# tfwcn/tensorflow2-machine-vision

Hardware: NVIDIA B200
Metric: images/sec (higher is better)
Workload: dtype f32

## Files before the change

### tensorflow2-machine-vision_b200/csrc/yolo_loss.cu

```cuda
#include "yolo_targets.cuh"
#include "exchange.cuh"

#define YL_LEVELS 3
#define YL_CHUNK 256
#define YL_ICHUNK 128

enum { YL_VARIANT_TF_YOLO_UTILS = 0, YL_VARIANT_KERAS_YOLO3 = 1 };

struct YlLevels {
  const float* y_true[YL_LEVELS];
  const float* y_pred[YL_LEVELS];
  int h[YL_LEVELS], w[YL_LEVELS], rec_per_img[YL_LEVELS], anchor_base[YL_LEVELS];
  int chunks_per_img[YL_LEVELS];
  int cta_base[YL_LEVELS + 1];
  int obj_chunks_per_img[YL_LEVELS];
  int obj_cta_base[YL_LEVELS + 1];
  uint32_t magic_w[YL_LEVELS];
  float anc_w[YL_LEVELS][8], anc_h[YL_LEVELS][8];
};

struct YlParams {
  YlLevels lv;
  int B, A, C, RF, n_img;
  float img_w, img_h;
  float thr;
  int metric, variant;
  float* obj_compact;
  float4* gt_box;
  float4* gt_aux;
  float log_thr;
  float logk[YL_LEVELS][8];
  float tmin_w[YL_LEVELS][8], tmin_h[YL_LEVELS][8];
  uint32_t magic_a;
  float* conf_grad;
  int32_t* obj_index;
  float inv_div;
  unsigned char* out_ignore;
  const float4* sp_t;
  const int32_t* sp_cls;
  const uint32_t* obj_bits;
  int bits_words;
  int32_t* gt_count;
  unsigned int* scan_ticket;
  uint32_t* pend_queue;
  unsigned int* pend_count;
  unsigned long long* obj_fixed;
  double* partials;
  double* partials_obj;
};

__device__ __forceinline__ void yl_locate(const YlLevels& lv, int cta, int& l, int& img, int& chunk) {
  l = 0;
#pragma unroll
  for (int k = 1; k < YL_LEVELS; ++k) if (cta >= lv.cta_base[k]) l = k;
  const int r = cta - lv.cta_base[l];
  img = r / lv.chunks_per_img[l];
  chunk = r - img * lv.chunks_per_img[l];
}

__device__ __forceinline__ bool yl_regular(const BoxT& b) {
  return (b.c2 > b.c0) && (b.c3 > b.c1) && (b.area > 0.0f) && (b.area < 3.0e38f) && (b.at == b.at) &&
         (dm_fabsf(b.c0) < 3.0e38f) && (dm_fabsf(b.c1) < 3.0e38f) && (dm_fabsf(b.c2) < 3.0e38f) && (dm_fabsf(b.c3) < 3.0e38f);
}

#define YL_OBJ_PER_THREAD 4
#define YL_OBJ_CHUNK (YL_CHUNK * YL_OBJ_PER_THREAD)

#define YL_SORT_CAP 2048
__device__ __forceinline__ void yl_gtprep_body(const YlParams& p, int l, int img, int* s_idx) {
  const int nthr = blockDim.x;
  const int rpi = p.lv.rec_per_img[l];
  const float* yt = p.sp_t ? nullptr : p.lv.y_true[l] + ((size_t)img * rpi) * p.RF;
  const int n = __ldcg(&p.gt_count[img * YL_LEVELS + l]);
  const size_t gbase = (size_t)img * p.n_img + p.lv.anchor_base[l];
  if (!p.sp_t && n > 1 && n <= YL_SORT_CAP) {
    for (int k = threadIdx.x; k < n; k += nthr) s_idx[k] = __ldcg(&p.obj_index[gbase + k]);
    __syncthreads();
    for (int k = threadIdx.x; k < n; k += nthr) {
      const int mine = s_idx[k];
      int rank = 0;
      for (int j = 0; j < n; ++j) rank += (s_idx[j] < mine) ? 1 : 0;
      p.obj_index[gbase + rank] = mine;
// ... 368 lines not shown
  if (n_gt > 0) {
    if (threadIdx.x == 0) s_nq = 0;
    if (threadIdx.x < YL_ICHUNK / 32) s_hit[threadIdx.x] = 0u;
    s_t[threadIdx.x] = make_float4(tx, ty, tw, th);
    __syncthreads();
    const YlFilter f = yl_filter_init(p, l, rin, active, tx, ty, tw, th);
    yl_filter_gts(f, gbox, gaux, n_gt, [&](int g, const float4 c, const float4 x, bool rejected) {
      if (!active | hit | rejected) return;
      const int slot = atomicAdd(&s_nq, 1);
      if (slot < YL_QCAP) s_q[slot] = (threadIdx.x << 24) | (uint32_t)g;
      else {
        float otx = tx, oty = ty, otw = tw, oth = th;
        asm volatile("" : "+f"(otx), "+f"(oty), "+f"(otw), "+f"(oth));
        if (yl_pair_hits(p, l, rin, otx, oty, otw, oth, c, x)) hit = true;
      }
    });
    if (hit) atomicOr(&s_hit[warp], 1u << lane);
    __syncthreads();
    const int nq = min(s_nq, YL_QCAP);
    for (int q = threadIdx.x; q < nq; q += YL_ICHUNK) {
      const uint32_t e = s_q[q];
      const int r = (int)(e >> 24), g = (int)(e & 0xffffffu);
      if ((s_hit[r >> 5] >> (r & 31)) & 1u) continue;
      const float4 t = s_t[r];
      if (yl_pair_hits(p, l, chunk * YL_ICHUNK + r, t.x, t.y, t.z, t.w, __ldg(gbox + g), __ldg(gaux + g)))
        atomicOr(&s_hit[r >> 5], 1u << (r & 31));
    }
    __syncthreads();
    hit = (s_hit[warp] >> lane) & 1u;
  }
  float e = 0.f;
  if (active) e = yl_record_term(p, l, img, p.lv.anchor_base[l] + rin, obj, pobj, hit, false);
  yl_store_partial(p, icta, e, s_acc);
}

#define YL_FIXED_ONE 4294967296.0

__global__ void __launch_bounds__(YL_ICHUNK, 10) yolo_loss_ignore_lean_kernel(YlParams p) {
  __shared__ double s_acc[YL_ICHUNK / 32];
  const int n_term_cta = YL_LEVELS * p.B * YL_TERM_SPLIT;
  const int n_icta = (int)gridDim.x - n_term_cta;
  if ((int)blockIdx.x >= n_icta) {
    __shared__ double s_tacc[YL_ICHUNK / 32][3];
    yl_terms_body(p, blockIdx.x - n_icta, s_tacc);
    return;
  }
  const int icta = blockIdx.x;
  int l, img, chunk;
  yl_locate(p.lv, icta, l, img, chunk);
  const int rpi = p.lv.rec_per_img[l];
  const int rin = chunk * YL_ICHUNK + (int)threadIdx.x;
  const int lane = threadIdx.x & 31;
  const bool active = rin < rpi;
  const int n_gt = p.gt_count[img * YL_LEVELS + l];
  const float4* gbox = p.gt_box + (size_t)img * p.n_img + p.lv.anchor_base[l];
  const float4* gaux = p.gt_aux + (size_t)img * p.n_img + p.lv.anchor_base[l];
  float obj = 0.f, tx = 0.f, ty = 0.f, tw = 0.f, th = 0.f, pobj = 0.f;
  if (active) {
    obj = yl_obj(p, img, p.lv.anchor_base[l] + rin);
    const size_t f0 = ((size_t)img * rpi + rin) * p.RF;
    const float4 lo = __ldcg(reinterpret_cast<const float4*>(p.lv.y_pred[l]) + (f0 >> 2));
    const float4 hi = __ldcg(reinterpret_cast<const float4*>(p.lv.y_pred[l]) + (f0 >> 2) + 1);
    yl_rotate5(lo, hi, (int)(f0 & 3), tx, ty, tw, th, pobj);
  }
  bool pending = false;
  if (n_gt > 0) {
    const YlFilter f = yl_filter_init(p, l, rin, active, tx, ty, tw, th);
    yl_filter_gts(f, gbox, gaux, n_gt, [&](int, const float4, const float4, bool rejected) { pending |= active & !rejected; });
  }
  {
    const uint32_t pm = __ballot_sync(0xffffffffu, pending);
    if (pm) {
      unsigned int base = 0;
      if (lane == 0) base = atomicAdd(p.pend_count, (unsigned int)__popc(pm));
      base = __shfl_sync(0xffffffffu, base, 0);
      if (pending) p.pend_queue[base + __popc(pm & ((1u << lane) - 1u))] = (uint32_t)((size_t)img * p.n_img + p.lv.anchor_base[l] + rin);
    }
  }
  float e = 0.f;
  if (active && !pending) e = yl_record_term(p, l, img, p.lv.anchor_base[l] + rin, obj, pobj, false, true);
  yl_store_partial(p, icta, e, s_acc);
}

__device__ __forceinline__ void yl_exact_pass(const YlParams& p, unsigned int gwarp, unsigned int nwarps) {
  const int lane = threadIdx.x & 31;
  const int half = lane >> 4, sub = lane & 15;
  const unsigned int n = *p.pend_count;
  for (unsigned int q0 = gwarp * 2u; q0 < n; q0 += nwarps * 2u) {
    const unsigned int q = q0 + (unsigned int)half;
    const bool valid = q < n;
    const uint32_t id = valid ? p.pend_queue[q] : 0u;
    const int img = (int)(id / (uint32_t)p.n_img);
    const int ain = (int)(id - (uint32_t)img * (uint32_t)p.n_img);
    int l = 0;
#pragma unroll
    for (int k = 1; k < YL_LEVELS; ++k) if (ain >= p.lv.anchor_base[k]) l = k;
    const int rin = ain - p.lv.anchor_base[l];
    const int rpi = p.lv.rec_per_img[l];
    const float* rec = p.lv.y_pred[l] + ((size_t)img * rpi + rin) * p.RF;
    const float tx = __ldg(rec), ty = __ldg(rec + 1), tw = __ldg(rec + 2), th = __ldg(rec + 3), pobj = __ldg(rec + 4);
    const float obj = yl_obj(p, img, ain);
    const int n_gt = valid ? p.gt_count[img * YL_LEVELS + l] : 0;
    const float4* gbox = p.gt_box + (size_t)img * p.n_img + p.lv.anchor_base[l];
    const float4* gaux = p.gt_aux + (size_t)img * p.n_img + p.lv.anchor_base[l];
    const BoxT pb = yl_decode_record(p, l, rin, tx, ty, tw, th);
    const bool pb_regular = yl_regular(pb);
    bool hit = false;
    for (int g0 = 0;; g0 += 16) {
      const bool more = g0 < n_gt && !hit;
      if (!__any_sync(0xffffffffu, more)) break;
      const int g = g0 + sub;
      bool h = false;
      if (more && g < n_gt) h = yl_box_hits(p, pb, pb_regular, __ldg(gbox + g), __ldg(gaux + g));
      const uint32_t bal = __ballot_sync(0xffffffffu, h);
      hit = hit || ((bal >> (16 * half)) & 0xffffu) != 0u;
    }
    if (valid && sub == 0) {
      const float e = yl_record_term(p, l, img, ain, obj, pobj, hit, false);
      if (e == e && e < 1.0e9f) atomicAdd(p.obj_fixed + l, (unsigned long long)((double)e * YL_FIXED_ONE + 0.5));
      else atomicOr(p.obj_fixed + l, 0x8000000000000000ull);
    }
  }
}

__global__ void __launch_bounds__(128) yolo_loss_ignore_exact_kernel(YlParams p) {
  yl_exact_pass(p, blockIdx.x * (blockDim.x >> 5) + (threadIdx.x >> 5), gridDim.x * (blockDim.x >> 5));
}

#define YL_FIN_CTAS 32
#define YL_FIN_THREADS 256

struct YlFinalize {
  const double* partials; const double* partials_obj;
  int cta_base[YL_LEVELS + 1]; int obj_cta_base[YL_LEVELS + 1];
  float batch_divisor; float* parts; float* loss;
  double* slices;
  unsigned int* ticket;
  B200Exchange xchg;
  const unsigned long long* obj_fixed;
  int publish_only;
};

__global__ void __launch_bounds__(YL_FIN_THREADS) yolo_loss_finalize_kernel(YlFinalize f, YlParams p, int exact) {
  __shared__ double s_red[YL_FIN_THREADS / 32][12];
  __shared__ bool s_last;
  if (exact) yl_exact_pass(p, blockIdx.x * (YL_FIN_THREADS / 32) + (threadIdx.x >> 5), gridDim.x * (YL_FIN_THREADS / 32));
  if ((int)blockIdx.x >= YL_FIN_CTAS) {
    __syncthreads();
    if (threadIdx.x == 0) { __threadfence(); s_last = (atomicAdd(f.ticket, 1u) == gridDim.x - 1); }
    __syncthreads();
    if (!s_last) return;
  } else {
  double acc[12];
#pragma unroll
  for (int i = 0; i < 12; ++i) acc[i] = 0.0;
  const int t0 = blockIdx.x * YL_FIN_THREADS + (int)threadIdx.x, stride = YL_FIN_CTAS * YL_FIN_THREADS;
#pragma unroll
  for (int l = 0; l < 3; ++l) {
#pragma unroll 4
    for (int c = f.cta_base[l] + t0; c < f.cta_base[l + 1]; c += stride) acc[l * 4 + 2] += f.partials[c];
    for (int c = f.obj_cta_base[l] + t0; c < f.obj_cta_base[l + 1]; c += stride) {
      acc[l * 4 + 0] += f.partials_obj[(size_t)c * 3 + 0];
      acc[l * 4 + 1] += f.partials_obj[(size_t)c * 3 + 1];
      acc[l * 4 + 3] += f.partials_obj[(size_t)c * 3 + 2];
    }
  }
  const int lane_ = threadIdx.x & 31, warp_ = threadIdx.x >> 5;
#pragma unroll
  for (int i = 0; i < 12; ++i) {
    double v = warp_sum_d(acc[i]);
    if (lane_ == 0) s_red[warp_][i] = v;
  }
  __syncthreads();
  if (threadIdx.x < 12) {
    double s = 0.0;
    for (int w = 0; w < YL_FIN_THREADS / 32; ++w) s += s_red[w][threadIdx.x];
    f.slices[blockIdx.x * 12 + threadIdx.x] = s;
    __threadfence();
  }
  __syncthreads();
  if (threadIdx.x == 0) { __threadfence(); s_last = (atomicAdd(f.ticket, 1u) == gridDim.x - 1); }
  __syncthreads();
  if (!s_last) return;
  }
  __threadfence();
  const int lane = threadIdx.x & 31, warp = threadIdx.x >> 5;
  if (warp == 0) {
    float v = 0.0f;
    if (lane < 12) {
      double s = 0.0;
      for (int g = 0; g < YL_FIN_CTAS; ++g) s += __ldcg(f.slices + g * 12 + lane);
      if (f.obj_fixed && (lane & 3) == 2) {
        const unsigned long long fx = __ldcg(f.obj_fixed + (lane >> 2));
        s += (fx >> 63) ? (double)__longlong_as_double(0x7ff8000000000000ll) : (double)fx * (1.0 / YL_FIXED_ONE);
      }
      v = DM_DIV((float)s, f.batch_divisor);
    }
    if (f.publish_only && f.xchg.world > 1) xchg_publish_warp<float>(f.xchg, v, 12);
    else v = xchg_allreduce_warp<float>(f.xchg, v, 12);
    if (lane < 12 && f.parts) f.parts[lane] = v;
    float total = 0.0f;
    for (int l = 0; l < 3; ++l) {
      const float t0_ = __shfl_sync(0xffffffffu, v, l * 4 + 0), t1 = __shfl_sync(0xffffffffu, v, l * 4 + 1);
      const float t2 = __shfl_sync(0xffffffffu, v, l * 4 + 2), t3 = __shfl_sync(0xffffffffu, v, l * 4 + 3);
      total = DM_ADD(total, DM_ADD(DM_ADD(DM_ADD(t0_, t1), t2), t3));
    }
    if (lane == 0) { *f.loss = total; *f.ticket = 0u; }
  }
}

struct YlGradDense {
  float* grad[YL_LEVELS];
  const float* conf_grad[YL_LEVELS];
  unsigned long long quads[YL_LEVELS];
  unsigned long long records[YL_LEVELS];
  int RF;
};

__global__ void __launch_bounds__(256) yolo_loss_grad_dense_kernel(YlGradDense g) {
  const int lane = threadIdx.x & 31;
  const unsigned long long total = g.quads[YL_LEVELS - 1];
  const unsigned long long wstride = (unsigned long long)gridDim.x * (blockDim.x >> 5);
  const int RF = g.RF;
  for (unsigned long long w = (unsigned long long)blockIdx.x * (blockDim.x >> 5) + (threadIdx.x >> 5); w < total; w += wstride) {
    unsigned long long q = w;
    const float* cg = g.conf_grad[0];
    float* gr = g.grad[0];
    if (w >= g.quads[1]) { q = w - g.quads[1]; cg = g.conf_grad[2]; gr = g.grad[2]; }
    else if (w >= g.quads[0]) { q = w - g.quads[0]; cg = g.conf_grad[1]; gr = g.grad[1]; }
    const float mine = (lane < 4) ? __ldg(cg + q * 4ull + lane) : 0.0f;
    const float c0 = __shfl_sync(0xffffffffu, mine, 0), c1 = __shfl_sync(0xffffffffu, mine, 1);
    const float c2 = __shfl_sync(0xffffffffu, mine, 2), c3 = __shfl_sync(0xffffffffu, mine, 3);
    float4* dst = reinterpret_cast<float4*>(gr) + q * (unsigned long long)RF;
    for (int j = lane; j < RF; j += 32) {
      const int e = 4 * j;
      float v[4];
#pragma unroll
      for (int k = 0; k < 4; ++k) {
        const int x = e + k - 4;
        v[k] = (x == 0) ? c0 : (x == RF) ? c1 : (x == 2 * RF) ? c2 : (x == 3 * RF) ? c3 : 0.0f;
      }
      __stcs(dst + j, make_float4(v[0], v[1], v[2], v[3]));
    }
  }
  if (blockIdx.x == 0) {
#pragma unroll
    for (int l = 0; l < YL_LEVELS; ++l) {
      const unsigned long long r0 = g.records[l] & ~3ull, n_tail = (g.records[l] - r0) * (unsigned long long)RF;
      for (unsigned long long t = threadIdx.x; t < n_tail; t += blockDim.x) {
        const unsigned long long rec = r0 + t / (unsigned long long)RF;
        const int c = (int)(t % (unsigned long long)RF);
        g.grad[l][r0 * (unsigned long long)RF + t] = (c == 4) ? g.conf_grad[l][rec] : 0.0f;
      }
    }
  }
}

#define YL_GRAD_SPLIT 8
__global__ void __launch_bounds__(256) yolo_loss_grad_objects_kernel(YlParams p, float* g0, float* g1, float* g2) {
  const int pair = blockIdx.x / YL_GRAD_SPLIT, split = blockIdx.x - pair * YL_GRAD_SPLIT;
  const int img = pair / YL_LEVELS, l = pair - img * YL_LEVELS;
  float* grad = (l == 0 ? g0 : l == 1 ? g1 : g2);
  const int n = p.gt_count[img * YL_LEVELS + l];
  const int rpi = p.lv.rec_per_img[l];
  const int lane = threadIdx.x & 31, warp = threadIdx.x >> 5;
  const int W = p.lv.w[l], H = p.lv.h[l];
  const float* yt = p.lv.y_true[l] + ((size_t)img * rpi) * p.RF;
  const float* yp = p.lv.y_pred[l] + ((size_t)img * rpi) * p.RF;
// ... 189 lines not shown
  for (int l = 0; l < YL_LEVELS; ++l)
    for (int a = 0; a < A; ++a)
    {
      p.logk[l][a] = (float)log(((double)p.lv.anc_w[l][a] * (double)p.lv.anc_h[l][a]) / ((double)img_w * (double)img_h));
      const double tw = log(4e-5 * (double)img_w / (double)p.lv.anc_w[l][a]);
      const double th = log(4e-5 * (double)img_h / (double)p.lv.anc_h[l][a]);
      p.tmin_w[l][a] = (float)(tw > -6.0 ? tw : -6.0);
      p.tmin_h[l][a] = (float)(th > -6.0 ? th : -6.0);
    }
  p.out_ignore = out_ignore;
  p.inv_div = 1.0f / batch_divisor;
  p.conf_grad = out_grad ? reinterpret_cast<float*>(wsb + ws.cgrad) : nullptr;
  p.obj_index = reinterpret_cast<int32_t*>(wsb + ws.oidx);
  p.magic_a = A == 1 ? 0u : (uint32_t)((1ull << 32) / (unsigned long long)A + 1ull);
  for (int l = 0; l < YL_LEVELS; ++l) p.lv.magic_w[l] = p.lv.w[l] == 1 ? 0u : (uint32_t)((1ull << 32) / (unsigned long long)p.lv.w[l] + 1ull);
  p.gt_count = reinterpret_cast<int32_t*>(wsb + ws.cnt);
  p.partials = reinterpret_cast<double*>(wsb + ws.part);
  p.partials_obj = reinterpret_cast<double*>(wsb + ws.part_obj);
  if (stages & 1) B200_CUDA(cudaMemsetAsync(wsb + ws.cnt, 0, ws.cnt_bytes, stream));
  p.pend_queue = reinterpret_cast<uint32_t*>(wsb + ws.pend);
  p.pend_count = reinterpret_cast<unsigned int*>(wsb + ws.cnt) + (size_t)B * YL_LEVELS + 1;
  p.obj_fixed = reinterpret_cast<unsigned long long*>(wsb + ws.cnt + b200_align_up(sizeof(int32_t) * ((size_t)B * YL_LEVELS + 2), 8));
  p.scan_ticket = (!sparse && (stages & 3) == 3) ? reinterpret_cast<unsigned int*>(p.obj_fixed + 3) : nullptr;
  p.sp_t = nullptr; p.sp_cls = nullptr; p.obj_bits = nullptr; p.bits_words = 0;
  if (sparse) {
    B200_REQUIRE(sparse->total_boxes >= 0 && sparse->offsets && sparse->assign_anchors_wh_host, B200_ERR_BAD_ARG, "b200_yolo_loss_from_boxes: null box arrays");
    B200_REQUIRE(sparse->total_boxes == 0 || (sparse->boxes && sparse->classes), B200_ERR_BAD_ARG, "b200_yolo_loss_from_boxes: null box arrays");
    B200_REQUIRE((reinterpret_cast<uintptr_t>(sparse->boxes) & 15) == 0, B200_ERR_BAD_ARG, "b200_yolo_loss_from_boxes: boxes not 16-byte aligned");
    YtParams t;
    B200_REQUIRE(yt_fill_geometry(t, A, C, sparse->assign_anchors_wh_host, image_wh_host, hw) == 0, B200_ERR_BAD_ARG, "b200_yolo_loss_from_boxes: bad geometry");
    t.boxes = sparse->boxes; t.classes = sparse->classes; t.offsets = sparse->offsets; t.B = B; t.total = sparse->total_boxes;
    p.bits_words = sws.bits_words;
    float4* sp_t = reinterpret_cast<float4*>(wsb + sws.sp_t);
    int32_t* sp_cls = reinterpret_cast<int32_t*>(wsb + sws.sp_cls);
    uint32_t* bits = reinterpret_cast<uint32_t*>(wsb + sws.bits);
    if (stages & 1) {
      B200_CUDA(cudaMemsetAsync(bits, 0, sizeof(uint32_t) * (size_t)B * sws.bits_words, stream));
      yolo_loss_assign_sparse_kernel<<<B, 128, 0, stream>>>(t, p, reinterpret_cast<int*>(wsb + sws.keys), sp_t, sp_cls, bits);
      B200_LAUNCH_CHECK();
    }
    p.sp_t = sp_t; p.sp_cls = sp_cls; p.obj_bits = bits;
  } else if (stages & 1) {
    yolo_loss_scan_kernel<<<ws.n_cta_obj, YL_CHUNK, 0, stream>>>(p);
    B200_LAUNCH_CHECK();
  }
  if ((stages & 2) && !p.scan_ticket) {
    yolo_loss_gtprep_kernel<<<YL_LEVELS * B, 128, 0, stream>>>(p);
    B200_LAUNCH_CHECK();
  }
  bool use_split = false;
  if (stages & 4) {
    cudaPointerAttributes attr;
    bool host_pred = false;
    if (cudaPointerGetAttributes(&attr, y_pred[YL_LEVELS - 1]) == cudaSuccess) host_pred = attr.type == cudaMemoryTypeHost;
    else (void)cudaGetLastError();
    const int grid = YL_LEVELS * B * YL_TERM_SPLIT + ws.n_cta;
    bool aligned16 = true;
    for (int l = 0; l < YL_LEVELS; ++l) aligned16 &= (reinterpret_cast<uintptr_t>(y_pred[l]) & 15) == 0;
    use_split = !host_pred && aligned16 && p.RF >= 8;
    if (use_split) {
      if (!(stages & 1)) B200_CUDA(cudaMemsetAsync(p.pend_count, 0, (size_t)(reinterpret_cast<unsigned char*>(p.obj_fixed + 3) - reinterpret_cast<unsigned char*>(p.pend_count)), stream));
      yolo_loss_ignore_lean_kernel<<<grid, YL_ICHUNK, 0, stream>>>(p);
      if (!(stages & 8)) {
        B200_LAUNCH_CHECK();
        yolo_loss_ignore_exact_kernel<<<1024, 128, 0, stream>>>(p);
      }
    } else {
      yolo_loss_ignore_kernel<<<grid, YL_ICHUNK, 0, stream>>>(p);
    }
    B200_LAUNCH_CHECK();
  }
  if (!(stages & 8)) return B200_OK;
  YlFinalize f;
  f.partials = p.partials; f.partials_obj = p.partials_obj;
  for (int l = 0; l <= YL_LEVELS; ++l) { f.cta_base[l] = p.lv.cta_base[l]; f.obj_cta_base[l] = l * B * YL_TERM_SPLIT; }
  f.batch_divisor = batch_divisor; f.parts = out_parts; f.loss = out_loss;
  f.slices = reinterpret_cast<double*>(wsb + ws.fin);
  f.ticket = reinterpret_cast<unsigned int*>(wsb + ws.cnt) + (size_t)B * YL_LEVELS;
  f.publish_only = publish_only;
  f.obj_fixed = p.obj_fixed;
  if (xchg) f.xchg = *xchg;
  else { f.xchg.rank = 0; f.xchg.world = 1; for (int r = 0; r < B200_XCHG_MAX_WORLD; ++r) f.xchg.mailbox[r] = nullptr; }
  int wide = 4 * b200_sm_count();
  if (wide < YL_FIN_CTAS) wide = YL_FIN_CTAS;
  yolo_loss_finalize_kernel<<<use_split ? wide : YL_FIN_CTAS, YL_FIN_THREADS, 0, stream>>>(f, p, use_split ? 1 : 0);
  B200_LAUNCH_CHECK();
  if (out_grad) {
    YlGradDense g;
    g.RF = p.RF;
    unsigned long long cum = 0;
    for (int l = 0; l < YL_LEVELS; ++l) {
      B200_REQUIRE(out_grad[l] && (reinterpret_cast<uintptr_t>(out_grad[l]) & 15) == 0, B200_ERR_BAD_ARG, "b200_yolo_loss_grad: grad level %d null or not 16-byte aligned", l);
      g.records[l] = (unsigned long long)B * p.lv.rec_per_img[l];
      g.grad[l] = out_grad[l];
      g.conf_grad[l] = p.conf_grad + (size_t)B * p.lv.anchor_base[l];
      cum += g.records[l] / 4ull;
      g.quads[l] = cum;
    }
    unsigned long long blocks = (cum + 7) / 8;
    const unsigned long long cap = (unsigned long long)b200_sm_count() * 64;
    if (blocks > cap) blocks = cap;
    if (blocks < 1) blocks = 1;
    yolo_loss_grad_dense_kernel<<<(int)blocks, 256, 0, stream>>>(g);
    B200_LAUNCH_CHECK();
    yolo_loss_grad_objects_kernel<<<B * YL_LEVELS * YL_GRAD_SPLIT, 256, 0, stream>>>(p, out_grad[0], out_grad[1], out_grad[2]);
    B200_LAUNCH_CHECK();
  }
  return B200_OK;
}

extern "C" int b200_yolo_loss(const float* const y_true[3], const float* const y_pred[3], const int32_t hw[6], int B,
                              int A, int C, const float* anchors_wh_host, const float* image_wh_host,
                              float iou_thresh, int metric, int variant, float batch_divisor, float* out_parts,
                              float* out_loss, unsigned char* out_ignore, void* workspace, size_t workspace_bytes,
                              void* stream_) {
  return yolo_loss_impl(y_true, y_pred, hw, B, A, C, anchors_wh_host, image_wh_host, iou_thresh, metric, variant,
                        batch_divisor, out_parts, out_loss, out_ignore, nullptr, workspace, workspace_bytes, stream_);
}

extern "C" int b200_yolo_loss_stages(const float* const y_true[3], const float* const y_pred[3], const int32_t hw[6], int B,
                                     int A, int C, const float* anchors_wh_host, const float* image_wh_host,
                                     float iou_thresh, int metric, int variant, float batch_divisor, float* out_parts,
                                     float* out_loss, void* workspace, size_t workspace_bytes, int stages, void* stream_) {
  B200_REQUIRE(stages > 0 && stages <= 0xf, B200_ERR_BAD_ARG, "b200_yolo_loss_stages: stages must be a non-empty subset of 0xf");
  return yolo_loss_impl(y_true, y_pred, hw, B, A, C, anchors_wh_host, image_wh_host, iou_thresh, metric, variant,
                        batch_divisor, out_parts, out_loss, nullptr, nullptr, workspace, workspace_bytes, stream_, nullptr, stages);
}

extern "C" size_t b200_yolo_loss_from_boxes_workspace_bytes(const int32_t hw[6], int B, int A, int total_boxes) {
  int n_img = 0;
  const YlWs w = yl_layout(hw, B, A, &n_img, nullptr);
  return yl_sparse_layout(w.total, B, n_img, total_boxes).total;
}

extern "C" int b200_yolo_loss_from_boxes(const float* boxes, const int32_t* classes, const int32_t* offsets, int total_boxes,
                                         const float* assign_anchors_wh_host, const float* const y_pred[3], const int32_t hw[6],
                                         int B, int A, int C, const float* anchors_wh_host, const float* image_wh_host,
                                         float iou_thresh, int metric, int variant, float batch_divisor, float* out_parts,
                                         float* out_loss, unsigned char* out_ignore, void* workspace, size_t workspace_bytes,
                                         void* stream_) {
  YlSparseIn sp;
  sp.boxes = boxes; sp.classes = classes; sp.offsets = offsets; sp.total_boxes = total_boxes;
  sp.assign_anchors_wh_host = assign_anchors_wh_host;
  return yolo_loss_impl(nullptr, y_pred, hw, B, A, C, anchors_wh_host, image_wh_host, iou_thresh, metric, variant,
                        batch_divisor, out_parts, out_loss, out_ignore, nullptr, workspace, workspace_bytes, stream_, &sp);
}

extern "C" int b200_yolo_loss_grad(const float* const y_true[3], const float* const y_pred[3], const int32_t hw[6],
                                   int B, int A, int C, const float* anchors_wh_host, const float* image_wh_host,
                                   float iou_thresh, int metric, int variant, float batch_divisor, float* out_parts,
                                   float* out_loss, float* const out_grad[3], void* workspace, size_t workspace_bytes,
                                   void* stream_) {
  B200_REQUIRE(out_grad, B200_ERR_BAD_ARG, "b200_yolo_loss_grad: null out_grad");
  return yolo_loss_impl(y_true, y_pred, hw, B, A, C, anchors_wh_host, image_wh_host, iou_thresh, metric, variant,
                        batch_divisor, out_parts, out_loss, nullptr, out_grad, workspace, workspace_bytes, stream_);
}

int b200_fill_exchange(B200Exchange& x, int rank, int world, void* const mailboxes[], const char* who);

extern "C" int b200_yolo_loss_dp(const float* const y_true[3], const float* const y_pred[3], const int32_t hw[6], int B,
                                 int A, int C, const float* anchors_wh_host, const float* image_wh_host,
                                 float iou_thresh, int metric, int variant, float global_batch, float* out_parts,
                                 float* out_loss, void* workspace, size_t workspace_bytes, int rank, int world,
                                 void* const mailboxes[], void* stream_) {
  B200Exchange x;
  const int rc = b200_fill_exchange(x, rank, world, mailboxes, "b200_yolo_loss_dp");
  if (rc != B200_OK) return rc;
// ... 47 lines not shown
```

### tensorflow2-machine-vision_b200/csrc/yolo_targets.cu

```cuda
#include "yolo_targets.cuh"

__global__ void fill_zero_kernel(float4* __restrict__ dst, size_t n_vec, float* __restrict__ tail, int n_tail) {
  const float4 z = make_float4(0.f, 0.f, 0.f, 0.f);
  size_t i = (size_t)blockIdx.x * blockDim.x + threadIdx.x;
  const size_t stride = (size_t)gridDim.x * blockDim.x;
#pragma unroll 4
  for (; i < n_vec; i += stride) __stcs(dst + i, z);
  if (blockIdx.x == 0 && (int)threadIdx.x < n_tail) tail[threadIdx.x] = 0.0f;
}

struct FillMulti {
  float4* dst[YT_LEVELS];
  unsigned long long n_vec[YT_LEVELS];
};

__global__ void fill_zero_multi_kernel(FillMulti f) {
  const float4 z = make_float4(0.f, 0.f, 0.f, 0.f);
  unsigned long long i = (unsigned long long)blockIdx.x * blockDim.x + threadIdx.x;
  const unsigned long long stride = (unsigned long long)gridDim.x * blockDim.x;
  const unsigned long long total = f.n_vec[YT_LEVELS - 1];
#pragma unroll 4
  for (; i < total; i += stride) {
    if (i < f.n_vec[0]) __stcs(f.dst[0] + i, z);
    else if (i < f.n_vec[1]) __stcs(f.dst[1] + (i - f.n_vec[0]), z);
    else __stcs(f.dst[2] + (i - f.n_vec[1]), z);
  }
}

__global__ void __launch_bounds__(128) yolo_scatter_targets_kernel(YtParams p) {
  const int img = blockIdx.x;
  const int beg = p.offsets[img], end = p.offsets[img + 1];
  const bool single = (end - beg) <= 128 * 4;
  for (int i0 = beg; i0 < end; i0 += 128 * 4) {
    float* recs[4];
#pragma unroll
    for (int u = 0; u < 4; ++u) {
      const int i = i0 + u * 128 + (int)threadIdx.x;
      recs[u] = nullptr;
      if (i < end) {
        float nx, ny, nw, nh;
        float* rec = yt_locate(p, img, i, nx, ny, nw, nh);
        recs[u] = rec;
        if (rec) {
          const float old = atomicAdd(rec + 4, 1.0f);
          if (old == 0.0f) {
            rec[0] = nx; rec[1] = ny; rec[2] = nw; rec[3] = nh;
            const int c = p.classes[i];
            if (c >= 0 && c < p.C) rec[5 + c] = 1.0f;
          }
        }
      }
    }
    __syncthreads();
    float cnt[4];
#pragma unroll
    for (int u = 0; u < 4; ++u) {
      float* rec = recs[u];
      cnt[u] = rec ? __ldcg(rec + 4) : 0.0f;
      if (cnt[u] > 1.0f) {
        for (int c = 0; c < p.RF; ++c) if (c != 4) rec[c] = 0.0f;
      }
    }
    __syncthreads();
    if (single) {
#pragma unroll
      for (int u = 0; u < 4; ++u) if (cnt[u] > 1.0f) recs[u][4] = 0.0f;
    }
  }
  if (single) return;
  for (int i = beg + (int)threadIdx.x; i < end; i += 128) {
    float nx, ny, nw, nh;
    float* rec = yt_locate(p, img, i, nx, ny, nw, nh);
    if (rec && rec[4] > 1.0f) rec[4] = 0.0f;
  }
}

__global__ void __launch_bounds__(128) yolo_reset_targets_kernel(YtParams p) {
  const int img = blockIdx.x, lane = threadIdx.x & 31, warp = threadIdx.x >> 5;
  const int beg = p.offsets[img], end = p.offsets[img + 1];
  for (int i0 = beg + warp * 32; i0 < end; i0 += 128) {
    float* mine = nullptr;
    if (i0 + lane < end) {
      float nx, ny, nw, nh;
      mine = yt_locate(p, img, i0 + lane, nx, ny, nw, nh);
    }
    const int n = min(32, end - i0);
    for (int k = 0; k < n; ++k) {
      float* rec = reinterpret_cast<float*>(__shfl_sync(0xffffffffu, reinterpret_cast<unsigned long long>(mine), k));
      if (rec) for (int c = lane; c < p.RF; c += 32) rec[c] = 0.0f;
    }
  }
}

extern "C" int b200_fill_zero(float* dst, size_t n, void* stream) {
  if (n == 0) return B200_OK;
  B200_REQUIRE(dst, B200_ERR_BAD_ARG, "b200_fill_zero: null pointer");
  B200_REQUIRE((reinterpret_cast<uintptr_t>(dst) & 15) == 0, B200_ERR_BAD_ARG, "b200_fill_zero: destination not 16-byte aligned");
  const size_t n_vec = n / 4;
  const int n_tail = (int)(n - n_vec * 4);
  size_t blocks = (n_vec + 255) / 256;
  const size_t cap = (size_t)b200_sm_count() * 128;
  if (blocks > cap) blocks = cap;
  if (blocks < 1) blocks = 1;
  fill_zero_kernel<<<(int)blocks, 256, 0, (cudaStream_t)stream>>>(reinterpret_cast<float4*>(dst), n_vec, dst + n_vec * 4, n_tail);
  B200_LAUNCH_CHECK();
  return B200_OK;
}

static int yt_fill_params(YtParams& p, const float* boxes, const int32_t* classes, const int32_t* offsets, int B, int total_boxes,
                          const float* anchors_wh_host, int A, const float* image_wh_host, int C, const int32_t hw[6],
                          float* const targets[3], const char* who) {
  B200_REQUIRE(B >= 0 && total_boxes >= 0 && A >= 1 && A <= 8 && C >= 0, B200_ERR_BAD_ARG, "%s: bad sizes", who);
  B200_REQUIRE(anchors_wh_host && image_wh_host && hw && targets, B200_ERR_BAD_ARG, "%s: null argument", who);
  p.boxes = boxes; p.classes = classes; p.offsets = offsets; p.B = B; p.total = total_boxes; p.A = A; p.C = C; p.RF = 5 + C;
  p.layers_num = YT_LEVELS;
  p.img_w = image_wh_host[0]; p.img_h = image_wh_host[1];
  for (int l = 0; l < YT_LEVELS; ++l) {
    B200_REQUIRE(targets[l] && hw[2 * l] > 0 && hw[2 * l + 1] > 0, B200_ERR_BAD_ARG, "%s: bad level %d", who, l);
    p.target[l] = targets[l]; p.h[l] = hw[2 * l]; p.w[l] = hw[2 * l + 1];
  }
  for (int k = 0; k < YT_LEVELS * A; ++k) { p.anc_w[k] = anchors_wh_host[2 * k]; p.anc_h[k] = anchors_wh_host[2 * k + 1]; }
  return B200_OK;
}

extern "C" int b200_yolo_reset_targets(const float* prev_boxes, const int32_t* prev_offsets, int B, int total_boxes,
                                       const float* anchors_wh_host, int A, const float* image_wh_host, int C,
                                       const int32_t hw[6], float* const targets[3], void* stream_) {
  YtParams p;
  const int st = yt_fill_params(p, prev_boxes, nullptr, prev_offsets, B, total_boxes, anchors_wh_host, A, image_wh_host, C, hw,
                                targets, "b200_yolo_reset_targets");
  if (st != B200_OK) return st;
  if (B == 0 || total_boxes == 0) return B200_OK;
  B200_REQUIRE(prev_boxes && prev_offsets, B200_ERR_BAD_ARG, "b200_yolo_reset_targets: null box arrays");
  B200_REQUIRE((reinterpret_cast<uintptr_t>(prev_boxes) & 15) == 0, B200_ERR_BAD_ARG, "b200_yolo_reset_targets: boxes not 16-byte aligned");
  yolo_reset_targets_kernel<<<B, 128, 0, (cudaStream_t)stream_>>>(p);
  B200_LAUNCH_CHECK();
  return B200_OK;
}

extern "C" int b200_yolo_assign_targets(const float* boxes, const int32_t* classes, const int32_t* offsets, int B,
                                        int total_boxes, const float* anchors_wh_host, int A, const float* image_wh_host,
                                        int C, const int32_t hw[6], float* const targets[3], int zero_fill, void* stream_) {
  cudaStream_t stream = (cudaStream_t)stream_;
  YtParams p;
  const int st0 = yt_fill_params(p, boxes, classes, offsets, B, total_boxes, anchors_wh_host, A, image_wh_host, C, hw, targets,
                                 "b200_yolo_assign_targets");
  if (st0 != B200_OK) return st0;
  if (B == 0) return B200_OK;
  if (zero_fill) {
    bool vec_ok = true;
    FillMulti f;
    unsigned long long cum = 0;
    for (int l = 0; l < YT_LEVELS; ++l) {
      const size_t n = (size_t)B * p.h[l] * p.w[l] * A * p.RF;
      vec_ok = vec_ok && (n % 4 == 0) && ((reinterpret_cast<uintptr_t>(targets[l]) & 15) == 0);
      f.dst[l] = reinterpret_cast<float4*>(targets[l]);
      cum += n / 4;
      f.n_vec[l] = cum;
    }
    if (vec_ok) {
      unsigned long long blocks = (cum + 255) / 256;
      const unsigned long long cap = (unsigned long long)b200_sm_count() * 128;
      if (blocks > cap) blocks = cap;
      if (blocks < 1) blocks = 1;
      fill_zero_multi_kernel<<<(int)blocks, 256, 0, stream>>>(f);
      B200_LAUNCH_CHECK();
    } else {
      for (int l = 0; l < YT_LEVELS; ++l) {
        int st = b200_fill_zero(targets[l], (size_t)B * p.h[l] * p.w[l] * A * p.RF, stream_);
        if (st != B200_OK) return st;
      }
    }
  }
  if (total_boxes > 0) {
    B200_REQUIRE(boxes && classes && offsets, B200_ERR_BAD_ARG, "b200_yolo_assign_targets: null box arrays");
    B200_REQUIRE((reinterpret_cast<uintptr_t>(boxes) & 15) == 0, B200_ERR_BAD_ARG, "b200_yolo_assign_targets: boxes not 16-byte aligned");
    yolo_scatter_targets_kernel<<<B, 128, 0, stream>>>(p);
    B200_LAUNCH_CHECK();
  }
  return B200_OK;
}
```

Baseline: 343,100.

## Overlap target scatter with zero-fill via PDL and split finalize exact pass

The target scatter kernel now uses programmatic dependent launch, so it computes assignments and detects duplicate cells with a shared-memory key comparison before waiting on the zero-fill. This replaces the atomic two-phase collision pass for images with at most 512 boxes. The finalize kernel now gives the exact-ignore pass only to the extra CTAs, letting the reduction CTAs proceed in parallel with it. It also processes two pending records per iteration to overlap their loads and uses an acq_rel atomic ticket in place of explicit fences. The risks are an O(n^2) key scan per image and subtle memory-ordering changes.

```diff
diff --git a/tensorflow2-machine-vision_b200/csrc/yolo_loss.cu b/tensorflow2-machine-vision_b200/csrc/yolo_loss.cu
--- a/tensorflow2-machine-vision_b200/csrc/yolo_loss.cu
+++ b/tensorflow2-machine-vision_b200/csrc/yolo_loss.cu
@@ -1,3 +1,5 @@
+#include <cuda/atomic>
+
 #include "yolo_targets.cuh"
 #include "exchange.cuh"
 
@@ -532,44 +534,62 @@
   yl_store_partial(p, icta, e, s_acc);
 }
 
+struct YlPending {
+  bool valid;
+  int img, l, ain, n_gt;
+  float tx, ty, tw, th, pobj, obj;
+};
+
+__device__ __forceinline__ YlPending yl_pending_load(const YlParams& p, unsigned int q, unsigned int n) {
+  YlPending r;
+  r.valid = q < n;
+  const uint32_t id = r.valid ? p.pend_queue[q] : 0u;
+  r.img = (int)(id / (uint32_t)p.n_img);
+  r.ain = (int)(id - (uint32_t)r.img * (uint32_t)p.n_img);
+  r.l = 0;
+#pragma unroll
+  for (int k = 1; k < YL_LEVELS; ++k) if (r.ain >= p.lv.anchor_base[k]) r.l = k;
+  const float* rec = p.lv.y_pred[r.l] + ((size_t)r.img * p.lv.rec_per_img[r.l] + (r.ain - p.lv.anchor_base[r.l])) * p.RF;
+  r.tx = __ldg(rec); r.ty = __ldg(rec + 1); r.tw = __ldg(rec + 2); r.th = __ldg(rec + 3); r.pobj = __ldg(rec + 4);
+  r.obj = yl_obj(p, r.img, r.ain);
+  r.n_gt = r.valid ? p.gt_count[r.img * YL_LEVELS + r.l] : 0;
+  return r;
+}
+
+__device__ __forceinline__ void yl_pending_resolve(const YlParams& p, const YlPending& r, int half, int sub) {
+  const int rin = r.ain - p.lv.anchor_base[r.l];
+  const float4* gbox = p.gt_box + (size_t)r.img * p.n_img + p.lv.anchor_base[r.l];
+  const float4* gaux = p.gt_aux + (size_t)r.img * p.n_img + p.lv.anchor_base[r.l];
+  const BoxT pb = yl_decode_record(p, r.l, rin, r.tx, r.ty, r.tw, r.th);
+  const bool pb_regular = yl_regular(pb);
+  bool hit = false;
+  for (int g0 = 0;; g0 += 16) {
+    const bool more = g0 < r.n_gt && !hit;
+    if (!__any_sync(0xffffffffu, more)) break;
+    const int g = g0 + sub;
+    bool h = false;
+    if (more && g < r.n_gt) h = yl_box_hits(p, pb, pb_regular, __ldg(gbox + g), __ldg(gaux + g));
+    const uint32_t bal = __ballot_sync(0xffffffffu, h);
+    hit = hit || ((bal >> (16 * half)) & 0xffffu) != 0u;
+  }
+  if (r.valid && sub == 0) {
+    const float e = yl_record_term(p, r.l, r.img, r.ain, r.obj, r.pobj, hit, false);
+    if (e == e && e < 1.0e9f) atomicAdd(p.obj_fixed + r.l, (unsigned long long)((double)e * YL_FIXED_ONE + 0.5));
+    else atomicOr(p.obj_fixed + r.l, 0x8000000000000000ull);
+  }
+}
+
 __device__ __forceinline__ void yl_exact_pass(const YlParams& p, unsigned int gwarp, unsigned int nwarps) {
   const int lane = threadIdx.x & 31;
   const int half = lane >> 4, sub = lane & 15;
   const unsigned int n = *p.pend_count;
-  for (unsigned int q0 = gwarp * 2u; q0 < n; q0 += nwarps * 2u) {
+  const unsigned int stride = nwarps * 2u;
+  for (unsigned int q0 = gwarp * 2u; q0 < n; q0 += 2u * stride) {
     const unsigned int q = q0 + (unsigned int)half;
-    const bool valid = q < n;
-    const uint32_t id = valid ? p.pend_queue[q] : 0u;
-    const int img = (int)(id / (uint32_t)p.n_img);
-    const int ain = (int)(id - (uint32_t)img * (uint32_t)p.n_img);
-    int l = 0;
-#pragma unroll
-    for (int k = 1; k < YL_LEVELS; ++k) if (ain >= p.lv.anchor_base[k]) l = k;
-    const int rin = ain - p.lv.anchor_base[l];
-    const int rpi = p.lv.rec_per_img[l];
-    const float* rec = p.lv.y_pred[l] + ((size_t)img * rpi + rin) * p.RF;
-    const float tx = __ldg(rec), ty = __ldg(rec + 1), tw = __ldg(rec + 2), th = __ldg(rec + 3), pobj = __ldg(rec + 4);
-    const float obj = yl_obj(p, img, ain);
-    const int n_gt = valid ? p.gt_count[img * YL_LEVELS + l] : 0;
-    const float4* gbox = p.gt_box + (size_t)img * p.n_img + p.lv.anchor_base[l];
-    const float4* gaux = p.gt_aux + (size_t)img * p.n_img + p.lv.anchor_base[l];
-    const BoxT pb = yl_decode_record(p, l, rin, tx, ty, tw, th);
-    const bool pb_regular = yl_regular(pb);
-    bool hit = false;
-    for (int g0 = 0;; g0 += 16) {
-      const bool more = g0 < n_gt && !hit;
-      if (!__any_sync(0xffffffffu, more)) break;
-      const int g = g0 + sub;
-      bool h = false;
-      if (more && g < n_gt) h = yl_box_hits(p, pb, pb_regular, __ldg(gbox + g), __ldg(gaux + g));
-      const uint32_t bal = __ballot_sync(0xffffffffu, h);
-      hit = hit || ((bal >> (16 * half)) & 0xffffu) != 0u;
-    }
-    if (valid && sub == 0) {
-      const float e = yl_record_term(p, l, img, ain, obj, pobj, hit, false);
-      if (e == e && e < 1.0e9f) atomicAdd(p.obj_fixed + l, (unsigned long long)((double)e * YL_FIXED_ONE + 0.5));
-      else atomicOr(p.obj_fixed + l, 0x8000000000000000ull);
-    }
+    const YlPending r0 = yl_pending_load(p, q, n);
+    const YlPending r1 = yl_pending_load(p, q + stride, n);
+    yl_pending_resolve(p, r0, half, sub);
+    if (__any_sync(0xffffffffu, r1.valid)) yl_pending_resolve(p, r1, half, sub);
   }
 }
 
@@ -594,12 +614,10 @@
 __global__ void __launch_bounds__(YL_FIN_THREADS) yolo_loss_finalize_kernel(YlFinalize f, YlParams p, int exact) {
   __shared__ double s_red[YL_FIN_THREADS / 32][12];
   __shared__ bool s_last;
-  if (exact) yl_exact_pass(p, blockIdx.x * (YL_FIN_THREADS / 32) + (threadIdx.x >> 5), gridDim.x * (YL_FIN_THREADS / 32));
   if ((int)blockIdx.x >= YL_FIN_CTAS) {
-    __syncthreads();
-    if (threadIdx.x == 0) { __threadfence(); s_last = (atomicAdd(f.ticket, 1u) == gridDim.x - 1); }
-    __syncthreads();
-    if (!s_last) return;
+    if (exact)
+      yl_exact_pass(p, (blockIdx.x - YL_FIN_CTAS) * (YL_FIN_THREADS / 32) + (threadIdx.x >> 5),
+                    (gridDim.x - YL_FIN_CTAS) * (YL_FIN_THREADS / 32));
   } else {
   double acc[12];
 #pragma unroll
@@ -626,14 +644,15 @@
     double s = 0.0;
     for (int w = 0; w < YL_FIN_THREADS / 32; ++w) s += s_red[w][threadIdx.x];
     f.slices[blockIdx.x * 12 + threadIdx.x] = s;
-    __threadfence();
-  }
-  __syncthreads();
-  if (threadIdx.x == 0) { __threadfence(); s_last = (atomicAdd(f.ticket, 1u) == gridDim.x - 1); }
+  }
+  }
+  __syncthreads();
+  if (threadIdx.x == 0) {
+    cuda::atomic_ref<unsigned int, cuda::thread_scope_device> ticket(*f.ticket);
+    s_last = ticket.fetch_add(1u, cuda::memory_order_acq_rel) == gridDim.x - 1;
+  }
   __syncthreads();
   if (!s_last) return;
-  }
-  __threadfence();
   const int lane = threadIdx.x & 31, warp = threadIdx.x >> 5;
   if (warp == 0) {
     float v = 0.0f;
@@ -989,7 +1008,7 @@
   if (xchg) f.xchg = *xchg;
   else { f.xchg.rank = 0; f.xchg.world = 1; for (int r = 0; r < B200_XCHG_MAX_WORLD; ++r) f.xchg.mailbox[r] = nullptr; }
   int wide = 4 * b200_sm_count();
-  if (wide < YL_FIN_CTAS) wide = YL_FIN_CTAS;
+  if (wide < 2 * YL_FIN_CTAS) wide = 2 * YL_FIN_CTAS;
   yolo_loss_finalize_kernel<<<use_split ? wide : YL_FIN_CTAS, YL_FIN_THREADS, 0, stream>>>(f, p, use_split ? 1 : 0);
   B200_LAUNCH_CHECK();
   if (out_grad) {
diff --git a/tensorflow2-machine-vision_b200/csrc/yolo_targets.cu b/tensorflow2-machine-vision_b200/csrc/yolo_targets.cu
--- a/tensorflow2-machine-vision_b200/csrc/yolo_targets.cu
+++ b/tensorflow2-machine-vision_b200/csrc/yolo_targets.cu
@@ -15,6 +15,7 @@
 };
 
 __global__ void fill_zero_multi_kernel(FillMulti f) {
+  asm volatile("griddepcontrol.launch_dependents;");
   const float4 z = make_float4(0.f, 0.f, 0.f, 0.f);
   unsigned long long i = (unsigned long long)blockIdx.x * blockDim.x + threadIdx.x;
   const unsigned long long stride = (unsigned long long)gridDim.x * blockDim.x;
@@ -27,10 +28,7 @@
   }
 }
 
-__global__ void __launch_bounds__(128) yolo_scatter_targets_kernel(YtParams p) {
-  const int img = blockIdx.x;
-  const int beg = p.offsets[img], end = p.offsets[img + 1];
-  const bool single = (end - beg) <= 128 * 4;
+__device__ __forceinline__ void yt_scatter_atomic(const YtParams& p, int img, int beg, int end) {
   for (int i0 = beg; i0 < end; i0 += 128 * 4) {
     float* recs[4];
 #pragma unroll
@@ -52,26 +50,69 @@
       }
     }
     __syncthreads();
-    float cnt[4];
 #pragma unroll
     for (int u = 0; u < 4; ++u) {
       float* rec = recs[u];
-      cnt[u] = rec ? __ldcg(rec + 4) : 0.0f;
-      if (cnt[u] > 1.0f) {
-        for (int c = 0; c < p.RF; ++c) if (c != 4) rec[c] = 0.0f;
-      }
+      if (rec && __ldcg(rec + 4) > 1.0f) for (int c = 0; c < p.RF; ++c) if (c != 4) rec[c] = 0.0f;
     }
     __syncthreads();
-    if (single) {
-#pragma unroll
-      for (int u = 0; u < 4; ++u) if (cnt[u] > 1.0f) recs[u][4] = 0.0f;
-    }
-  }
-  if (single) return;
+  }
   for (int i = beg + (int)threadIdx.x; i < end; i += 128) {
     float nx, ny, nw, nh;
     float* rec = yt_locate(p, img, i, nx, ny, nw, nh);
     if (rec && rec[4] > 1.0f) rec[4] = 0.0f;
+  }
+}
+
+#define YT_KEYS 512
+
+__global__ void __launch_bounds__(128) yolo_scatter_targets_kernel(YtParams p) {
+  __shared__ __align__(16) int s_key[YT_KEYS];
+  const int img = blockIdx.x;
+  const int beg = p.offsets[img], end = p.offsets[img + 1];
+  const int n = end - beg;
+  if (n > YT_KEYS) {
+    asm volatile("griddepcontrol.wait;" ::: "memory");
+    yt_scatter_atomic(p, img, beg, end);
+    return;
+  }
+  const int base1 = p.h[0] * p.w[0] * p.A, base2 = base1 + p.h[1] * p.w[1] * p.A;
+  const int rounds = (n + 127) / 128;
+  float* recs[4];
+  float4 v[4];
+  int cls[4], key[4];
+#pragma unroll
+  for (int u = 0; u < 4; ++u) {
+    const int k = u * 128 + (int)threadIdx.x;
+    recs[u] = nullptr;
+    key[u] = -2;
+    if (u < rounds) {
+      int layer, rin;
+      if (k < n && yt_assign(p, beg + k, layer, rin, v[u].x, v[u].y, v[u].z, v[u].w)) {
+        key[u] = (layer == 0 ? 0 : layer == 1 ? base1 : base2) + rin;
+        recs[u] = p.target[layer] + ((size_t)img * p.h[layer] * p.w[layer] * p.A + rin) * p.RF;
+        cls[u] = p.classes[beg + k];
+      }
+      s_key[k] = recs[u] ? key[u] : -1;
+    }
+  }
+  __syncthreads();
+  int hits[4] = {0, 0, 0, 0};
+#pragma unroll 4
+  for (int j = 0; j < n; j += 4) {
+    const int4 kk = *reinterpret_cast<const int4*>(s_key + j);
+#pragma unroll
+    for (int u = 0; u < 4; ++u)
+      if (u < rounds) hits[u] += (kk.x == key[u]) + (kk.y == key[u]) + (kk.z == key[u]) + (kk.w == key[u]);
+  }
+  asm volatile("griddepcontrol.wait;" ::: "memory");
+#pragma unroll
+  for (int u = 0; u < 4; ++u) {
+    float* rec = recs[u];
+    if (rec && hits[u] == 1) {
+      rec[0] = v[u].x; rec[1] = v[u].y; rec[2] = v[u].z; rec[3] = v[u].w; rec[4] = 1.0f;
+      if (cls[u] >= 0 && cls[u] < p.C) rec[5 + cls[u]] = 1.0f;
+    }
   }
 }
 
@@ -147,6 +188,7 @@
                                  "b200_yolo_assign_targets");
   if (st0 != B200_OK) return st0;
   if (B == 0) return B200_OK;
+  bool after_own_fill = false;
   if (zero_fill) {
     bool vec_ok = true;
     FillMulti f;
@@ -165,6 +207,7 @@
       if (blocks < 1) blocks = 1;
       fill_zero_multi_kernel<<<(int)blocks, 256, 0, stream>>>(f);
       B200_LAUNCH_CHECK();
+      after_own_fill = true;
     } else {
       for (int l = 0; l < YT_LEVELS; ++l) {
         int st = b200_fill_zero(targets[l], (size_t)B * p.h[l] * p.w[l] * A * p.RF, stream_);
@@ -175,8 +218,13 @@
   if (total_boxes > 0) {
     B200_REQUIRE(boxes && classes && offsets, B200_ERR_BAD_ARG, "b200_yolo_assign_targets: null box arrays");
     B200_REQUIRE((reinterpret_cast<uintptr_t>(boxes) & 15) == 0, B200_ERR_BAD_ARG, "b200_yolo_assign_targets: boxes not 16-byte aligned");
-    yolo_scatter_targets_kernel<<<B, 128, 0, stream>>>(p);
-    B200_LAUNCH_CHECK();
-  }
-  return B200_OK;
-}
+    cudaLaunchConfig_t cfg = {};
+    cfg.gridDim = dim3((unsigned)B); cfg.blockDim = dim3(128); cfg.dynamicSmemBytes = 0; cfg.stream = stream;
+    cudaLaunchAttribute attr[1];
+    attr[0].id = cudaLaunchAttributeProgrammaticStreamSerialization;
+    attr[0].val.programmaticStreamSerializationAllowed = 1;
+    cfg.attrs = attr; cfg.numAttrs = after_own_fill ? 1 : 0;
+    B200_CUDA(cudaLaunchKernelEx(&cfg, yolo_scatter_targets_kernel, p));
+  }
+  return B200_OK;
+}
```

Result: no change. 342,700 (median of 6 runs) (-0.1%).
